# Scalsol/mega.pytorch

Measured on AMD Instinct MI355X. Metric: frames/sec MEGA R-101 inference, 1000x600 VID clip, higher is better.
Workload: dtype bf16

## Files before the change

### include/mega_hip.h

```cpp
#ifndef MEGA_HIP_H
#define MEGA_HIP_H

#include <stddef.h>

#ifdef __cplusplus
extern "C" {
#endif

#define MEGA_F32 0
#define MEGA_BF16 1
#define MEGA_F16 2

#define MEGA_OK 0
#define MEGA_ERR_ARG 1
#define MEGA_ERR_LAUNCH 2
#define MEGA_ERR_WS 3
#define MEGA_ERR_LIMIT 4

int mega_conv2d_nhwc(const void* in, const void* w, const float* scale, const float* bias, const void* residual,
                     void* out, int N, int H, int W, int Cin, int Cout, int R, int S, int stride, int pad, int dil,
                     int relu, int ldo, int ldr, int in_dtype, int out_dtype, void* stream);
int mega_conv2d_nhwc_tile(int M, int Cout, int K);
int mega_conv2d_nhwc_plan(int M, int Cout, int K, int in_dtype);
int mega_conv2d_nhwc_plan_ex(int N, int H, int W, int Cin, int Cout, int R, int S, int stride, int pad, int dil, int ldo,
                             int has_residual, int in_dtype, int out_dtype);

size_t mega_conv2d_nhwc_workspace_bytes(int M, int Cout, int K);
int mega_conv2d_nhwc_ws(const void* in, const void* w, const float* scale, const float* bias, const void* residual,
                        void* out, int N, int H, int W, int Cin, int Cout, int R, int S, int stride, int pad, int dil,
                        int relu, int ldo, int ldr, int in_dtype, int out_dtype, void* ws, size_t ws_bytes, void* stream);

int mega_stem_conv_bn_relu(const float* in, const float* w_tap64, const float* scale, const float* bias, void* out,
                           int N, int H, int W, int out_dtype, void* stream);
int mega_stem_conv_bn_relu_bf16(const float* in, const void* w_n176_bf16, const float* scale, const float* bias,
                                void* out, int N, int H, int W, void* stream);
int mega_stem_conv_bn_relu_bf16_u8(const void* frames_u8, const void* w_n176_bf16, const float* scale, const float* bias,
                                   void* out, int N, int H, int W, float mean0, float mean1, float mean2, int to_bgr,
                                   void* stream);

int mega_stem_pool_dt(const void* in, int u8, const void* w_n176, const float* scale, const float* bias, void* out, int N,
                      int H, int W, float mean0, float mean1, float mean2, int to_bgr, int dtype, void* stream);

int mega_maxpool3x3s2_nhwc(const void* in, void* out, int N, int H, int W, int C, int dtype, void* stream);

int mega_avgpool2x2_ceil_nhwc(const void* in, void* out, int N, int H, int W, int C, int dtype, void* stream);

int mega_roi_align_fwd(const void* feat, const float* rois, void* out, int K, int C, int H, int W,
                       float spatial_scale, int pooled_h, int pooled_w, int sampling_ratio, int in_nhwc,
                       int out_nhwc, int dtype, int out_dtype, void* stream);

size_t mega_nms_full_workspace_bytes(int n);
int mega_nms(const float* dets, const float* scores, int n, float thr, int strict_gt, long long* keep_out,
             int* keep_cnt, void* ws, size_t ws_bytes, void* stream);

size_t mega_nms_workspace_bytes(int P, int nmax);
int mega_nms_sorted(const float* boxes, const int* counts, const unsigned char* valid, const int* order, int P,
                    int nmax, float thr, int strict_gt, int max_keep, int* keep_pos, int* keep_cnt,
                    unsigned char* flags, void* ws, size_t ws_bytes, void* stream);

size_t mega_rpn_select_workspace_bytes(int B, int pre_nms_top_n);
int mega_rpn_select_idx(const float* rpn_out, const float* cell_anchors, int B, int Hf, int Wf, int A, int ldc,
                        int anchor_stride, int pre_nms_top_n, int post_nms_top_n, float nms_thresh, int strict_gt,
                        float min_size, float im_w, float im_h, float* proposals, float* prop_scores, int* prop_cnt,
                        int* prop_index, void* ws, size_t ws_bytes, void* stream);

size_t mega_postprocess_workspace_bytes(int R, int NC);
int mega_postprocess(const float* logits, const float* deltas, const float* props, const int* nprop, int R, int NC,
                     float wx, float wy, float ww, float wh, float im_w, float im_h, float score_thresh,
                     float nms_thresh, int strict_gt, int max_det, float* out_boxes, float* out_scores,
                     long long* out_labels, int* out_cnt, float* probs_out, void* ws, size_t ws_bytes,
                     void* stream);

size_t mega_postprocess_batched_workspace_bytes(int B, int R, int NC);
int mega_postprocess_batched(const float* logits, const float* deltas, const float* props, const int* nprop, int B,
// ... 164 lines not shown
```

### mega/pytorch_amd/_lib.py

```python
import ctypes
import os

HERE = os.path.dirname(os.path.abspath(__file__))
LIB_PATH = os.path.join(HERE, "libmega_hip.so")

c_int, c_float, c_void_p, c_size_t = ctypes.c_int, ctypes.c_float, ctypes.c_void_p, ctypes.c_size_t
c_longlong = ctypes.c_longlong

_ERR = {1: "bad argument", 2: "kernel launch failure", 3: "workspace too small", 4: "kernel loop bound exceeded"}

SIGNATURES = {
    "mega_conv2d_nhwc": (c_int, [c_void_p] * 6 + [c_int] * 15 + [c_void_p]),
    "mega_conv2d_nhwc_ws": (c_int, [c_void_p] * 6 + [c_int] * 15 + [c_void_p, c_size_t, c_void_p]),
    "mega_conv2d_nhwc_workspace_bytes": (c_size_t, [c_int] * 3),
    "mega_stem_conv_bn_relu": (c_int, [c_void_p] * 5 + [c_int] * 4 + [c_void_p]),
    "mega_stem_conv_bn_relu_bf16": (c_int, [c_void_p] * 5 + [c_int] * 3 + [c_void_p]),
    "mega_stem_conv_bn_relu_bf16_u8": (c_int, [c_void_p] * 5 + [c_int] * 3 + [c_float] * 3 + [c_int, c_void_p]),
    "mega_stem_pool_dt": (c_int, [c_void_p, c_int] + [c_void_p] * 4 + [c_int] * 3 + [c_float] * 3 + [c_int, c_int, c_void_p]),
    "mega_maxpool3x3s2_nhwc": (c_int, [c_void_p] * 2 + [c_int] * 5 + [c_void_p]),
    "mega_avgpool2x2_ceil_nhwc": (c_int, [c_void_p] * 2 + [c_int] * 5 + [c_void_p]),
    "mega_roi_align_fwd": (c_int, [c_void_p] * 3 + [c_int] * 4 + [c_float] + [c_int] * 7 + [c_void_p]),
    "mega_nms_full_workspace_bytes": (c_size_t, [c_int]),
    "mega_nms": (c_int, [c_void_p, c_void_p, c_int, c_float, c_int, c_void_p, c_void_p, c_void_p, c_size_t, c_void_p]),
    "mega_nms_workspace_bytes": (c_size_t, [c_int, c_int]),
    "mega_nms_sorted": (c_int, [c_void_p] * 4 + [c_int, c_int, c_float, c_int, c_int] + [c_void_p] * 4 +
                        [c_size_t, c_void_p]),
    "mega_rpn_select_workspace_bytes": (c_size_t, [c_int, c_int]),
    "mega_rpn_select_idx": (c_int, [c_void_p, c_void_p] + [c_int] * 8 + [c_float, c_int, c_float, c_float, c_float] +
                            [c_void_p] * 5 + [c_size_t, c_void_p]),
    "mega_postprocess_workspace_bytes": (c_size_t, [c_int, c_int]),
    "mega_postprocess": (c_int, [c_void_p] * 4 + [c_int, c_int] + [c_float] * 8 + [c_int, c_int] + [c_void_p] * 6 +
                         [c_size_t, c_void_p]),
    "mega_postprocess_batched_workspace_bytes": (c_size_t, [c_int, c_int, c_int]),
    "mega_postprocess_batched": (c_int, [c_void_p] * 4 + [c_int, c_int, c_int] + [c_float] * 8 + [c_int, c_int] +
                                 [c_void_p] * 6 + [c_size_t, c_void_p]),
    "mega_postprocess_candidates_batched": (c_int, [c_void_p] * 4 + [c_int] * 3 + [c_float] * 7 + [c_void_p] * 3),
    "mega_bbox_aug_merge_workspace_bytes": (c_size_t, [c_int] * 4),
    "mega_bbox_aug_merge": (c_int, [c_void_p, c_void_p] + [c_int] * 4 + [c_void_p] * 3 + [c_float, c_float, c_int, c_int] +
                            [c_void_p] * 5 + [c_size_t, c_void_p]),
    "mega_soft_merge_workspace_bytes": (c_size_t, [c_int] * 4),
    "mega_soft_merge": (c_int, [c_void_p, c_void_p] + [c_int] * 4 + [c_void_p] * 3 +
                        [c_float, c_float, c_int, c_int, c_float, c_int, c_float, c_int, c_int] + [c_void_p] * 5 +
                        [c_size_t, c_void_p]),
    "mega_position_logits": (c_int, [c_void_p] * 6 + [c_int] * 4 + [c_void_p]),
    "mega_relation_attention_splits": (c_int, [c_int, c_int, c_int]),
    "mega_relation_attention_workspace_bytes": (c_size_t, [c_int, c_int, c_int]),
    "mega_relation_attention": (c_int, [c_void_p, c_int, c_void_p, c_int, c_void_p, c_int, c_void_p, c_int,
                                        c_void_p, c_int, c_void_p, c_void_p, c_int, c_int, c_int, c_int, c_float,
                                        c_int, c_void_p, c_size_t, c_void_p]),
    "mega_relation_attention_batched": (c_int, [c_void_p, c_int, c_int, c_float, c_int, c_void_p]),
    "mega_position_logits_tiled_dt": (c_int, [c_void_p] * 6 + [c_int] * 3 + [c_void_p]),
# ... 80 lines not shown
```

### mega/pytorch_amd/csrc/spatial.hip

```cpp
#include "common.h"

namespace {

constexpr int ST_T = 16;
constexpr int ST_P = ST_T * 2 + 5;
constexpr int ST_PW = ST_P + 1;

template <typename OT>
__global__ __launch_bounds__(256) void stem_conv_kernel(const float* __restrict__ in, const float* __restrict__ w,
                                                        const float* __restrict__ scale,
                                                        const float* __restrict__ bias, OT* __restrict__ out, int N,
                                                        int H, int W, int Ho, int Wo) {
  __shared__ float patch[3][ST_P][ST_PW];
  const int tid = threadIdx.x;
  const int n = blockIdx.z;
  const int oy0 = blockIdx.y * ST_T, ox0 = blockIdx.x * ST_T;
  const int iy0 = oy0 * 2 - 3, ix0 = ox0 * 2 - 3;
  for (int e = tid; e < 3 * ST_P * ST_P; e += 256) {
    const int c = e / (ST_P * ST_P);
    const int rem = e - c * ST_P * ST_P;
    const int y = rem / ST_P, x = rem - y * ST_P;
    const int iy = iy0 + y, ix = ix0 + x;
    float v = 0.f;
    if ((unsigned)iy < (unsigned)H && (unsigned)ix < (unsigned)W) v = in[((size_t)(n * 3 + c) * H + iy) * W + ix];
// ... 524 lines not shown
    for (int i = 0; i < 2; ++i)
#pragma unroll
      for (int j = 0; j < 2; ++j)
        acc[i][j] = __builtin_amdgcn_mfma_f32_32x32x16_bf16(__builtin_bit_cast(bf16x8_t, a[i]),
                                                            __builtin_bit_cast(bf16x8_t, b[j]), acc[i][j], 0, 0, 0);
  }
  __syncthreads();
#pragma unroll
  for (int j = 0; j < 2; ++j) {
    const int ch = j * 32 + p;
    const float sc = scale[ch], bi = bias[ch];
#pragma unroll
    for (int i = 0; i < 2; ++i) {
#pragma unroll
      for (int r = 0; r < 16; ++r) {
        const int px = (r & 3) + 8 * (r >> 2) + 4 * half;
        *reinterpret_cast<unsigned short*>(smem + ((2 * wave + i) * SM_TX + px) * SM_OUT_PS + ch * 2) =
            (bf16_t)(f32_to_bf16(fmaxf(acc[i][j][r] * sc + bi, 0.f)) & 0x7fffu);
      }
    }
  }
  __syncthreads();
#pragma unroll
  for (int i = 0; i < SM_TY * SM_TX * 8 / 256; ++i) {
    const int v = tid + 256 * i;
    const int pl = v >> 3, cv = v & 7;
    const int oy = oy0 + pl / SM_TX, ox = ox0 + pl % SM_TX;
    if (oy < Ho && ox < Wo)
      *reinterpret_cast<uint4*>(out + (((size_t)n * Ho + oy) * Wo + ox) * 64 + cv * 8) =
          *reinterpret_cast<const uint4*>(smem + pl * SM_OUT_PS + cv * 16);
  }
}

constexpr int SP_PY = 4, SP_PX = 16;
constexpr int SP_TY = 2 * SP_PY + 1, SP_TX = 2 * SP_PX + 1;
constexpr int SP_NPIX = SP_TY * SP_TX;
constexpr int SP_NBLK = (SP_NPIX + 31) / 32;
constexpr int SP_PH = 2 * SP_TY + 5, SP_PW = 2 * SP_TX + 5, SP_PS = 72;
static_assert(SP_PW + 1 <= SP_PS, "the zero-weight 8th tap reads one column past the patch");

__host__ __device__ constexpr int sp_group_off(int g) {
  const int gg = g < 21 ? g : 20;
  return (gg / 7) * (SP_PH * SP_PS) + (gg % 7) * SP_PS;
}

template <bool U8, typename HT = bf16_t>
__global__ __launch_bounds__(256, 3) void stem_pool_kernel(const void* __restrict__ in_, const bf16_t* __restrict__ w,
                                                        const float* __restrict__ scale, const float* __restrict__ bias,
                                                        bf16_t* __restrict__ out, int N, int H, int W, int Ho, int Wo, int Hp,
                                                        int Wp, float m0, float m1, float m2, int to_bgr) {
  const float* __restrict__ in = reinterpret_cast<const float*>(in_);
  const unsigned char* __restrict__ in8 = reinterpret_cast<const unsigned char*>(in_);
  constexpr int PATCH_B = (3 * SP_PH * SP_PS * 2 + 15) / 16 * 16, OUT_PS = 144;
  constexpr int LDS_B = SP_NBLK * 32 * OUT_PS > PATCH_B + 64 * SM_WS * 2 ? SP_NBLK * 32 * OUT_PS : PATCH_B + 64 * SM_WS * 2;
  __shared__ __attribute__((aligned(16))) unsigned char smem[LDS_B];
  unsigned short* patch = reinterpret_cast<unsigned short*>(smem);
  unsigned short* wl = reinterpret_cast<unsigned short*>(smem + PATCH_B);
  const int tid = threadIdx.x, lane = tid & 63, wave = tid >> 6;
  const int n = blockIdx.z;
  const int py0 = blockIdx.y * SP_PY, px0 = blockIdx.x * SP_PX;
  const int oy0 = 2 * py0 - 1, ox0 = 2 * px0 - 1;
  const int iy0 = oy0 * 2 - 3, ix0 = ox0 * 2 - 3;
  constexpr int NPL = (3 * SP_PH * SP_PS + 255) / 256, NWL = (64 * (SM_K / 8) + 255) / 256;
  float pv[NPL];
  u32x4_t wv[NWL];
#pragma unroll
  for (int i = 0; i < NPL; ++i) {
    const int e = tid + 256 * i;
    const int c = e / (SP_PH * SP_PS);
    const int rem = e - c * (SP_PH * SP_PS);
    const int y = rem / SP_PS, x = rem - y * SP_PS;
    const int iy = iy0 + y, ix = ix0 + x;
    pv[i] = 0.f;
    if (e < 3 * SP_PH * SP_PS && x < SP_PW && (unsigned)iy < (unsigned)H && (unsigned)ix < (unsigned)W) {
      if (U8) {
        const float mean = c == 0 ? m0 : (c == 1 ? m1 : m2);
        pv[i] = (float)in8[(((size_t)n * H + iy) * W + ix) * 3 + (to_bgr ? 2 - c : c)] - mean;
      } else {
        pv[i] = in[((size_t)(n * 3 + c) * H + iy) * W + ix];
      }
    }
  }
#pragma unroll
  for (int i = 0; i < NWL; ++i) {
    const int e = tid + 256 * i;
    const int row = e / (SM_K / 8), v = e - row * (SM_K / 8);
    if (e < 64 * (SM_K / 8)) wv[i] = *reinterpret_cast<const u32x4_t*>(w + row * SM_K + v * 8);
  }
#pragma unroll
  for (int i = 0; i < NPL; ++i) {
    const int e = tid + 256 * i;
    if (e < 3 * SP_PH * SP_PS) patch[e] = Half16<HT>::cvt(pv[i]);
  }
#pragma unroll
  for (int i = 0; i < NWL; ++i) {
    const int e = tid + 256 * i;
    const int row = e / (SM_K / 8), v = e - row * (SM_K / 8);
    if (e < 64 * (SM_K / 8)) *reinterpret_cast<u32x4_t*>(&wl[row * SM_WS + v * 8]) = wv[i];
  }
  __syncthreads();

  const int p = lane & 31, half = lane >> 5;
  constexpr int NB = 3;
  f32x16_t acc[NB][2];
  int pbase[NB];
#pragma unroll
  for (int b = 0; b < NB; ++b) {
    const int pix = min(32 * (wave + 4 * b) + p, SP_NPIX - 1);
    const int r = pix / SP_TX, c = pix - r * SP_TX;
    pbase[b] = 2 * r * SP_PS + 2 * c;
#pragma unroll
    for (int j = 0; j < 2; ++j)
#pragma unroll
      for (int q = 0; q < 16; ++q) acc[b][j][q] = 0.f;
  }
#pragma unroll
  for (int ks = 0; ks < SM_K / 16; ++ks) {
    u32x4_t bfr[2];
#pragma unroll
    for (int j = 0; j < 2; ++j) bfr[j] = *reinterpret_cast<const u32x4_t*>(&wl[(j * 32 + p) * SM_WS + ks * 16 + half * 8]);
#pragma unroll
    for (int b = 0; b < NB; ++b) {
      if (wave + 4 * b < SP_NBLK) {
        const unsigned* base = reinterpret_cast<const unsigned*>(patch + pbase[b] + (half ? sp_group_off(2 * ks + 1) : sp_group_off(2 * ks)));
        const u32x4_t a = {base[0], base[1], base[2], base[3]};
#pragma unroll
        for (int j = 0; j < 2; ++j) acc[b][j] = Half16<HT>::mfma32(a, bfr[j], acc[b][j]);
      }
    }
  }
  __syncthreads();
#pragma unroll
  for (int j = 0; j < 2; ++j) {
    const int ch = j * 32 + p;
    const float sc = scale[ch], bi = bias[ch];
#pragma unroll
    for (int b = 0; b < NB; ++b) {
      if (wave + 4 * b < SP_NBLK) {
#pragma unroll
        for (int q = 0; q < 16; ++q) {
          const int pix = 32 * (wave + 4 * b) + (q & 3) + 8 * (q >> 2) + 4 * half;
          const int r = pix / SP_TX, c = pix - r * SP_TX;
          const int oy = oy0 + r, ox = ox0 + c;
          const bool ok = pix < SP_NPIX && (unsigned)oy < (unsigned)Ho && (unsigned)ox < (unsigned)Wo;
          const unsigned short hv = (unsigned short)(Half16<HT>::cvt(fmaxf(acc[b][j][q] * sc + bi, 0.f)) & 0x7fffu);
          *reinterpret_cast<unsigned short*>(smem + pix * OUT_PS + ch * 2) = ok ? hv : (unsigned short)0;
        }
      }
    }
  }
  __syncthreads();
#pragma unroll
  for (int i = 0; i < SP_PY * SP_PX * 8 / 256; ++i) {
    const int v = tid + 256 * i;
    const int pl = v >> 3, cv = v & 7;
    const int ty = pl / SP_PX, tx = pl - ty * SP_PX;
    const int oy = py0 + ty, ox = px0 + tx;
    typedef unsigned short u16x8_t __attribute__((ext_vector_type(8)));
    u16x8_t m = {0, 0, 0, 0, 0, 0, 0, 0};
#pragma unroll
    for (int dy = 0; dy < 3; ++dy)
#pragma unroll
      for (int dx = 0; dx < 3; ++dx) {
        const u16x8_t q = *reinterpret_cast<const u16x8_t*>(smem + ((2 * ty + dy) * SP_TX + 2 * tx + dx) * OUT_PS + cv * 16);
        m = __builtin_elementwise_max(m, q);
      }
    if (oy < Hp && ox < Wp) *reinterpret_cast<u16x8_t*>(out + (((size_t)n * Hp + oy) * Wp + ox) * 64 + cv * 8) = m;
  }
}

}

extern "C" int mega_stem_conv_bn_relu_bf16(const float* in, const void* w_n176_bf16, const float* scale,
                                           const float* bias, void* out, int N, int H, int W, void* stream) {
  mega_clear_error();
  if (!in || !w_n176_bf16 || !scale || !bias || !out || N <= 0 || H <= 0 || W <= 0) return MEGA_ERR_ARG;
  const int Ho = (H + 6 - 7) / 2 + 1, Wo = (W + 6 - 7) / 2 + 1;
  dim3 grid(cdiv(Wo, SM_TX), cdiv(Ho, SM_TY), N);
  hipLaunchKernelGGL(stem_mfma_kernel<false>, grid, dim3(256), 0, (hipStream_t)stream, (const void*)in,
                     (const bf16_t*)w_n176_bf16, scale, bias, (bf16_t*)out, N, H, W, Ho, Wo, 0.f, 0.f, 0.f, 0);
  return mega_check_launch();
}

extern "C" int mega_stem_conv_bn_relu_bf16_u8(const void* frames_u8, const void* w_n176_bf16, const float* scale,
                                              const float* bias, void* out, int N, int H, int W, float mean0, float mean1,
                                              float mean2, int to_bgr, void* stream) {
  mega_clear_error();
  if (!frames_u8 || !w_n176_bf16 || !scale || !bias || !out || N <= 0 || H <= 0 || W <= 0) return MEGA_ERR_ARG;
  const int Ho = (H + 6 - 7) / 2 + 1, Wo = (W + 6 - 7) / 2 + 1;
  dim3 grid(cdiv(Wo, SM_TX), cdiv(Ho, SM_TY), N);
  hipLaunchKernelGGL(stem_mfma_kernel<true>, grid, dim3(256), 0, (hipStream_t)stream, frames_u8, (const bf16_t*)w_n176_bf16,
                     scale, bias, (bf16_t*)out, N, H, W, Ho, Wo, mean0, mean1, mean2, to_bgr);
  return mega_check_launch();
}

extern "C" int mega_stem_conv_bn_relu(const float* in, const float* w_tap64, const float* scale, const float* bias,
                                      void* out, int N, int H, int W, int out_dtype, void* stream) {
  mega_clear_error();
  if (!in || !w_tap64 || !scale || !bias || !out || N <= 0 || H <= 0 || W <= 0) return MEGA_ERR_ARG;
  const int Ho = (H + 6 - 7) / 2 + 1, Wo = (W + 6 - 7) / 2 + 1;
// ... 100 lines not shown
                       (bf16_t*)out, K, C, H, W, spatial_scale, pooled_h, pooled_w, sampling_ratio, in_nhwc, out_nhwc);
  else if (dtype == MEGA_F16 && out_dtype == MEGA_F16)
    hipLaunchKernelGGL((roi_align_kernel<f16_t, f16_t>), grid, dim3(threads), 0, st, (const f16_t*)feat, rois,
                       (f16_t*)out, K, C, H, W, spatial_scale, pooled_h, pooled_w, sampling_ratio, in_nhwc, out_nhwc);
  else if (dtype == MEGA_F32 && out_dtype == MEGA_F32)
    hipLaunchKernelGGL((roi_align_kernel<float, float>), grid, dim3(threads), 0, st, (const float*)feat, rois,
                       (float*)out, K, C, H, W, spatial_scale, pooled_h, pooled_w, sampling_ratio, in_nhwc, out_nhwc);
  else
    return MEGA_ERR_ARG;
  return mega_check_launch();
}

extern "C" int mega_avgpool2x2_ceil_nhwc(const void* in, void* out, int N, int H, int W, int C, int dtype,
                                         void* stream) {
  mega_clear_error();
  if (!in || !out || N <= 0 || H <= 0 || W <= 0 || C <= 0) return MEGA_ERR_ARG;
  const int Ho = (H + 1) / 2, Wo = (W + 1) / 2;
  hipStream_t st = (hipStream_t)stream;
  const int ve = dtype == MEGA_BF16 ? 8 : 4;
  if (C % ve) return MEGA_ERR_ARG;
  const size_t total = (size_t)N * Ho * Wo * (C / ve);
  const int blocks = (int)((total + 255) / 256 > 8192 ? 8192 : (total + 255) / 256);
  if (dtype == MEGA_BF16)
    hipLaunchKernelGGL((avgpool2_kernel<bf16_t>), dim3(blocks), dim3(256), 0, st, (const bf16_t*)in, (bf16_t*)out, N, H,
                       W, C, Ho, Wo);
  else if (dtype == MEGA_F32)
    hipLaunchKernelGGL((avgpool2_kernel<float>), dim3(blocks), dim3(256), 0, st, (const float*)in, (float*)out, N, H, W,
                       C, Ho, Wo);
  else
    return MEGA_ERR_ARG;
  return mega_check_launch();
}

extern "C" int mega_stem_pool_dt(const void* in, int u8, const void* w_n176, const float* scale, const float* bias,
                                 void* out, int N, int H, int W, float mean0, float mean1, float mean2, int to_bgr,
                                 int dtype, void* stream) {
  mega_clear_error();
  if (!in || !w_n176 || !scale || !bias || !out || N <= 0 || H <= 0 || W <= 0) return MEGA_ERR_ARG;
  if (dtype != MEGA_BF16 && dtype != MEGA_F16) return MEGA_ERR_ARG;
  const int Ho = (H + 6 - 7) / 2 + 1, Wo = (W + 6 - 7) / 2 + 1;
  const int Hp = (Ho + 2 - 3) / 2 + 1, Wp = (Wo + 2 - 3) / 2 + 1;
  dim3 grid(cdiv(Wp, SP_PX), cdiv(Hp, SP_PY), N);
  hipStream_t st = (hipStream_t)stream;
  const bf16_t* w = (const bf16_t*)w_n176;
  bf16_t* o = (bf16_t*)out;
  if (!u8) { mean0 = mean1 = mean2 = 0.f; to_bgr = 0; }
  if (dtype == MEGA_F16) {
    if (u8) hipLaunchKernelGGL((stem_pool_kernel<true, f16_t>), grid, dim3(256), 0, st, in, w, scale, bias, o, N, H, W, Ho, Wo, Hp, Wp, mean0, mean1, mean2, to_bgr);
    else hipLaunchKernelGGL((stem_pool_kernel<false, f16_t>), grid, dim3(256), 0, st, in, w, scale, bias, o, N, H, W, Ho, Wo, Hp, Wp, mean0, mean1, mean2, to_bgr);
  } else {
    if (u8) hipLaunchKernelGGL((stem_pool_kernel<true, bf16_t>), grid, dim3(256), 0, st, in, w, scale, bias, o, N, H, W, Ho, Wo, Hp, Wp, mean0, mean1, mean2, to_bgr);
    else hipLaunchKernelGGL((stem_pool_kernel<false, bf16_t>), grid, dim3(256), 0, st, in, w, scale, bias, o, N, H, W, Ho, Wo, Hp, Wp, mean0, mean1, mean2, to_bgr);
  }
  return mega_check_launch();
}

extern "C" int mega_roi_align_fwd_planes_dt(const float* feat, const float* rois, void* out, int K, int C, int H, int W,
                                            float spatial_scale, int pooled_h, int pooled_w, int sampling_ratio, int dtype,
                                            void* stream) {
  mega_clear_error();
  if (K == 0) return MEGA_OK;
  if (dtype != MEGA_BF16 && dtype != MEGA_F16) return MEGA_ERR_ARG;
  if (!feat || !rois || !out || K < 0 || C <= 0 || C % 4 || H <= 0 || W <= 0 || pooled_h <= 0 || pooled_w <= 0) return MEGA_ERR_ARG;
  const int CV = C / 4;
  const long long total = (long long)K * pooled_h * pooled_w * CV;
  const bool sliced = CV % 8 == 0 && CV / 8 >= 16 && total / 8 >= 256 * 64;
  long long nb = ((sliced ? total / 8 : total) + 255) / 256;
  if (nb > 131072) nb = 131072;
  dim3 vgrid((unsigned)(sliced ? nb * 8 : nb));
  hipStream_t st = (hipStream_t)stream;
  const bool separable = sliced && sampling_ratio <= 0 && pooled_w <= RS_MAXPW && pooled_h <= RS_MAXPW;
  if (separable) {
    if (dtype == MEGA_F16)
      hipLaunchKernelGGL((roi_align_nhwc_sep_kernel<float, 8, true, f16_t>), dim3((unsigned)(K * 8)), dim3(256), 0, st, feat, rois,
                         (float*)out, K, C, H, W, spatial_scale, pooled_h, pooled_w);
    else
      hipLaunchKernelGGL((roi_align_nhwc_sep_kernel<float, 8, true, bf16_t>), dim3((unsigned)(K * 8)), dim3(256), 0, st, feat, rois,
                         (float*)out, K, C, H, W, spatial_scale, pooled_h, pooled_w);
    return mega_check_launch();
  }
  if (dtype == MEGA_F16) {
    if (sliced)
      hipLaunchKernelGGL((roi_align_nhwc_vec_kernel<float, true, true, f16_t>), vgrid, dim3(256), 0, st, feat, rois, (float*)out, K, C,
                         H, W, spatial_scale, pooled_h, pooled_w, sampling_ratio);
    else
      hipLaunchKernelGGL((roi_align_nhwc_vec_kernel<float, false, true, f16_t>), vgrid, dim3(256), 0, st, feat, rois, (float*)out, K,
                         C, H, W, spatial_scale, pooled_h, pooled_w, sampling_ratio);
// ... 10 lines not shown
```

### mega/pytorch_amd/ops.py

```python
import contextlib
import ctypes
import threading
import math

import torch

from . import _lib

F32, BF16, F16 = 0, 1, 2
_DT = {torch.float32: F32, torch.bfloat16: BF16, torch.float16: F16}
_HALF = (torch.bfloat16, torch.float16)


def _dt(t):
    try:
        return _DT[t.dtype]
    except KeyError:
        raise TypeError("unsupported dtype %s (float32 / bfloat16 / float16 only)" % t.dtype)


_LAUNCH = threading.local()


def _stream():
# ... 289 lines not shown
    assert C == 3 and x_nchw.dtype == torch.float32 and x_nchw.is_contiguous()
    Ho, Wo = (H - 1) // 2 + 1, (W - 1) // 2 + 1
    out = torch.empty((N, Ho, Wo, 64), dtype=out_dtype, device=x_nchw.device)
    _tok = _pb("stem", 2.0 * N * Ho * Wo * 64 * 147, x_nchw.numel() * 4 + out.numel() * out.element_size())
    if out_dtype == torch.bfloat16 and w_n160 is not None:
        _gpu(w_n160)
        assert w_n160.dtype == torch.bfloat16 and tuple(w_n160.shape) == (64, 176) and w_n160.is_contiguous()
        rc = lib.mega_stem_conv_bn_relu_bf16(_ptr(x_nchw), _ptr(w_n160), _ptr(scale), _ptr(bias), _ptr(out), N, H, W,
                                             _stream())
    else:
        rc = lib.mega_stem_conv_bn_relu(_ptr(x_nchw), _ptr(w_tap64), _ptr(scale), _ptr(bias), _ptr(out), N, H, W,
                                        _DT[out_dtype], _stream())
    _pe(_tok)
    _lib.check(rc, "mega_stem_conv_bn_relu")
    return out


def stem_u8(frames_u8, w_n160, scale, bias, mean, to_bgr=True):
    _gpu(frames_u8, w_n160, scale, bias)
    lib = _lib.load()
    N, H, W, C = frames_u8.shape
    assert C == 3 and frames_u8.dtype == torch.uint8 and frames_u8.is_contiguous()
    assert w_n160.dtype == torch.bfloat16 and tuple(w_n160.shape) == (64, 176) and w_n160.is_contiguous()
    Ho, Wo = (H - 1) // 2 + 1, (W - 1) // 2 + 1
    out = torch.empty((N, Ho, Wo, 64), dtype=torch.bfloat16, device=frames_u8.device)
    _tok = _pb("stem", 2.0 * N * Ho * Wo * 64 * 147, frames_u8.numel() + out.numel() * 2)
    rc = lib.mega_stem_conv_bn_relu_bf16_u8(_ptr(frames_u8), _ptr(w_n160), _ptr(scale), _ptr(bias), _ptr(out), N, H, W,
                                            float(mean[0]), float(mean[1]), float(mean[2]), int(to_bgr), _stream())
    _pe(_tok)
    _lib.check(rc, "mega_stem_conv_bn_relu_bf16_u8")
    return out


def stem_pool(x, w_n160, scale, bias, mean=None, to_bgr=True):
    _gpu(x, w_n160, scale, bias)
    lib = _lib.load()
    u8 = x.dtype == torch.uint8
    if u8:
        N, H, W, C = x.shape
        assert mean is not None
    else:
        N, C, H, W = x.shape
        assert x.dtype == torch.float32
        mean = (0.0, 0.0, 0.0)
    assert C == 3 and x.is_contiguous()
    assert w_n160.dtype in _HALF and tuple(w_n160.shape) == (64, 176) and w_n160.is_contiguous()
    Ho, Wo = (H - 1) // 2 + 1, (W - 1) // 2 + 1
    Hp, Wp = (Ho - 1) // 2 + 1, (Wo - 1) // 2 + 1
    out = torch.empty((N, Hp, Wp, 64), dtype=w_n160.dtype, device=x.device)
    _tok = _pb("stem", 2.0 * N * Ho * Wo * 64 * 147, x.numel() * x.element_size() + out.numel() * 2)
    rc = lib.mega_stem_pool_dt(_ptr(x), int(u8), _ptr(w_n160), _ptr(scale), _ptr(bias), _ptr(out), N, H, W,
                               float(mean[0]), float(mean[1]), float(mean[2]), int(to_bgr), _dt(w_n160), _stream())
    _pe(_tok)
    _lib.check(rc, "mega_stem_pool_dt")
    return out


def pack_stem_weight_bf16(w_oihw, dtype=torch.bfloat16):
    w = torch.zeros((64, 22, 8), dtype=torch.float32, device=w_oihw.device)
    w[:, :21, :7] = w_oihw.detach().float().reshape(64, 21, 7)
    w = w.reshape(64, 176)
    return w.to(dtype).contiguous()


def maxpool3x3s2(x):
    _gpu(x)
    lib = _lib.load()
    N, H, W, C = x.shape
    assert x.is_contiguous()
    Ho, Wo = (H - 1) // 2 + 1, (W - 1) // 2 + 1
    out = torch.empty((N, Ho, Wo, C), dtype=x.dtype, device=x.device)
    _tok = _pb("maxpool", 0.0, (x.numel() + out.numel()) * x.element_size())
    rc = lib.mega_maxpool3x3s2_nhwc(_ptr(x), _ptr(out), N, H, W, C, _dt(x), _stream())
    _pe(_tok)
    _lib.check(rc, "mega_maxpool3x3s2_nhwc")
    return out


def roi_align(feat, rois, spatial_scale, pooled, sampling_ratio, in_nhwc=True, out_nhwc=True):
    _gpu(feat, rois)
    lib = _lib.load()
    if in_nhwc:
        B, H, W, C = feat.shape
    else:
        B, C, H, W = feat.shape
    ph, pw = pooled
    K = rois.shape[0]
# ... 995 lines not shown
```

Before: 903.0.

## Make fused stem conv+maxpool persistent with double-buffered patch prefetch

Turns the fused stem conv/BN/ReLU/maxpool kernel into a persistent grid sized to twice the CU count. Each block loops over tiles and prefetches the next tile's input patch into a second LDS buffer while running MFMA on the current one. It also reshapes tiles to 7x8 pooled outputs, uses 16-byte vector loads with byte alignment for uint8 frames, keeps scale and bias in LDS, and reserves separate LDS regions for the patch and output staging. The cost is more dynamic LDS per block, which caps occupancy at two blocks per CU, plus more complex boundary handling. The stem is only a small part of the R-101 MEGA pipeline, so its effect on the end-to-end rate is limited.

```diff
diff --git a/include/mega_hip.h b/include/mega_hip.h
--- a/include/mega_hip.h
+++ b/include/mega_hip.h
@@ -40,6 +40,9 @@
 
 int mega_stem_pool_dt(const void* in, int u8, const void* w_n176, const float* scale, const float* bias, void* out, int N,
                       int H, int W, float mean0, float mean1, float mean2, int to_bgr, int dtype, void* stream);
+int mega_stem_pool_dt_grid(const void* in, int u8, const void* w_n176, const float* scale, const float* bias, void* out, int N,
+                           int H, int W, float mean0, float mean1, float mean2, int to_bgr, int dtype, int max_blocks,
+                           void* stream);
 
 int mega_maxpool3x3s2_nhwc(const void* in, void* out, int N, int H, int W, int C, int dtype, void* stream);
 
diff --git a/mega/pytorch_amd/_lib.py b/mega/pytorch_amd/_lib.py
--- a/mega/pytorch_amd/_lib.py
+++ b/mega/pytorch_amd/_lib.py
@@ -17,6 +17,7 @@
     "mega_stem_conv_bn_relu_bf16": (c_int, [c_void_p] * 5 + [c_int] * 3 + [c_void_p]),
     "mega_stem_conv_bn_relu_bf16_u8": (c_int, [c_void_p] * 5 + [c_int] * 3 + [c_float] * 3 + [c_int, c_void_p]),
     "mega_stem_pool_dt": (c_int, [c_void_p, c_int] + [c_void_p] * 4 + [c_int] * 3 + [c_float] * 3 + [c_int, c_int, c_void_p]),
+    "mega_stem_pool_dt_grid": (c_int, [c_void_p, c_int] + [c_void_p] * 4 + [c_int] * 3 + [c_float] * 3 + [c_int, c_int, c_int, c_void_p]),
     "mega_maxpool3x3s2_nhwc": (c_int, [c_void_p] * 2 + [c_int] * 5 + [c_void_p]),
     "mega_avgpool2x2_ceil_nhwc": (c_int, [c_void_p] * 2 + [c_int] * 5 + [c_void_p]),
     "mega_roi_align_fwd": (c_int, [c_void_p] * 3 + [c_int] * 4 + [c_float] + [c_int] * 7 + [c_void_p]),
diff --git a/mega/pytorch_amd/csrc/spatial.hip b/mega/pytorch_amd/csrc/spatial.hip
--- a/mega/pytorch_amd/csrc/spatial.hip
+++ b/mega/pytorch_amd/csrc/spatial.hip
@@ -580,140 +580,250 @@
   }
 }
 
-constexpr int SP_PY = 4, SP_PX = 16;
+constexpr int SP_PY = 7, SP_PX = 8;
 constexpr int SP_TY = 2 * SP_PY + 1, SP_TX = 2 * SP_PX + 1;
 constexpr int SP_NPIX = SP_TY * SP_TX;
 constexpr int SP_NBLK = (SP_NPIX + 31) / 32;
-constexpr int SP_PH = 2 * SP_TY + 5, SP_PW = 2 * SP_TX + 5, SP_PS = 72;
+constexpr int SP_NB = SP_NBLK / 4;
+static_assert(SP_NBLK % 4 == 0, "the MFMA blocks divide evenly over the four waves");
+constexpr int SP_PH = 2 * SP_TY + 5, SP_PW = 2 * SP_TX + 5, SP_PS = 40;
 static_assert(SP_PW + 1 <= SP_PS, "the zero-weight 8th tap reads one column past the patch");
+static_assert(SP_PS % 4 == 0, "a patch row is whole 4-pixel groups");
+constexpr int SP_GR = SP_PS / 4, SP_NIT = SP_PH * SP_GR;
+constexpr int SP_NEL = 3 * SP_PH * SP_PS;
+constexpr int SP_PATCH_B = SP_NEL * 2, SP_OUT_PS = 144;
+static_assert(SP_PATCH_B % 16 == 0, "patch buffers stay 16-byte aligned");
+constexpr int SP_OFF_SC = 64 * SM_WS * 2, SP_OFF_BI = SP_OFF_SC + 256, SP_OFF_P = SP_OFF_BI + 256;
+constexpr int SP_OFF_ST = SP_OFF_P + 2 * SP_PATCH_B, SP_LDS = SP_OFF_ST + SP_NBLK * 32 * SP_OUT_PS;
+static_assert(SP_OFF_P % 16 == 0 && SP_OFF_ST % 16 == 0, "16-byte LDS vectors");
+constexpr int SP_BLOCKS_PER_CU = 2;
+static_assert(SP_BLOCKS_PER_CU * SP_LDS <= 160 * 1024, "two blocks per CU");
 
 __host__ __device__ constexpr int sp_group_off(int g) {
   const int gg = g < 21 ? g : 20;
   return (gg / 7) * (SP_PH * SP_PS) + (gg % 7) * SP_PS;
 }
 
+typedef unsigned int u32x2_t __attribute__((ext_vector_type(2)));
+
 template <bool U8, typename HT = bf16_t>
-__global__ __launch_bounds__(256, 3) void stem_pool_kernel(const void* __restrict__ in_, const bf16_t* __restrict__ w,
-                                                        const float* __restrict__ scale, const float* __restrict__ bias,
-                                                        bf16_t* __restrict__ out, int N, int H, int W, int Ho, int Wo, int Hp,
-                                                        int Wp, float m0, float m1, float m2, int to_bgr) {
+__global__ __launch_bounds__(256, SP_BLOCKS_PER_CU) void stem_pool_kernel(
+    const void* __restrict__ in_, long long in_bytes, const bf16_t* __restrict__ w, const float* __restrict__ scale,
+    const float* __restrict__ bias, bf16_t* __restrict__ out, int N, int H, int W, int Ho, int Wo, int Hp, int Wp, float m0,
+    float m1, float m2, int to_bgr, int tiles_y, int tiles_x, int tiles) {
   const float* __restrict__ in = reinterpret_cast<const float*>(in_);
   const unsigned char* __restrict__ in8 = reinterpret_cast<const unsigned char*>(in_);
-  constexpr int PATCH_B = (3 * SP_PH * SP_PS * 2 + 15) / 16 * 16, OUT_PS = 144;
-  constexpr int LDS_B = SP_NBLK * 32 * OUT_PS > PATCH_B + 64 * SM_WS * 2 ? SP_NBLK * 32 * OUT_PS : PATCH_B + 64 * SM_WS * 2;
-  __shared__ __attribute__((aligned(16))) unsigned char smem[LDS_B];
-  unsigned short* patch = reinterpret_cast<unsigned short*>(smem);
-  unsigned short* wl = reinterpret_cast<unsigned short*>(smem + PATCH_B);
+  extern __shared__ __attribute__((aligned(16))) unsigned char sp_smem[];
+  unsigned short* wl = reinterpret_cast<unsigned short*>(sp_smem);
+  const float* lsc = reinterpret_cast<const float*>(sp_smem + SP_OFF_SC);
+  const float* lbi = reinterpret_cast<const float*>(sp_smem + SP_OFF_BI);
+  unsigned char* stage = sp_smem + SP_OFF_ST;
   const int tid = threadIdx.x, lane = tid & 63, wave = tid >> 6;
-  const int n = blockIdx.z;
-  const int py0 = blockIdx.y * SP_PY, px0 = blockIdx.x * SP_PX;
-  const int oy0 = 2 * py0 - 1, ox0 = 2 * px0 - 1;
-  const int iy0 = oy0 * 2 - 3, ix0 = ox0 * 2 - 3;
-  constexpr int NPL = (3 * SP_PH * SP_PS + 255) / 256, NWL = (64 * (SM_K / 8) + 255) / 256;
-  float pv[NPL];
-  u32x4_t wv[NWL];
-#pragma unroll
-  for (int i = 0; i < NPL; ++i) {
-    const int e = tid + 256 * i;
-    const int c = e / (SP_PH * SP_PS);
-    const int rem = e - c * (SP_PH * SP_PS);
-    const int y = rem / SP_PS, x = rem - y * SP_PS;
-    const int iy = iy0 + y, ix = ix0 + x;
-    pv[i] = 0.f;
-    if (e < 3 * SP_PH * SP_PS && x < SP_PW && (unsigned)iy < (unsigned)H && (unsigned)ix < (unsigned)W) {
-      if (U8) {
-        const float mean = c == 0 ? m0 : (c == 1 ? m1 : m2);
-        pv[i] = (float)in8[(((size_t)n * H + iy) * W + ix) * 3 + (to_bgr ? 2 - c : c)] - mean;
-      } else {
-        pv[i] = in[((size_t)(n * 3 + c) * H + iy) * W + ix];
-      }
-    }
-  }
-#pragma unroll
-  for (int i = 0; i < NWL; ++i) {
+  const int p = lane & 31, half = lane >> 5;
+  const int mis = (int)(reinterpret_cast<uintptr_t>(in_) & 3);
+
+  auto origin = [&](int t, int& n, int& py0, int& px0) {
+    n = t / (tiles_y * tiles_x);
+    const int r = t - n * (tiles_y * tiles_x);
+    const int ty = r / tiles_x;
+    py0 = ty * SP_PY;
+    px0 = (r - ty * tiles_x) * SP_PX;
+  };
+  auto ld_bytes = [&](long long o) -> unsigned {
+    unsigned v = 0;
+#pragma unroll
+    for (int b = 0; b < 4; ++b)
+      if (o + b >= 0 && o + b < in_bytes) v |= (unsigned)in8[o + b] << (8 * b);
+    return v;
+  };
+
+  constexpr int NRAW = U8 ? 8 : (SP_NEL + 255) / 256;
+  constexpr int NRAWV = (NRAW + 3) / 4;
+  auto load_raw = [&](int t, u32x4_t (&raw)[NRAWV]) {
+    int n, py0, px0;
+    origin(t, n, py0, px0);
+    const int iy0 = 4 * py0 - 5, ix0 = 4 * px0 - 5;
+    if constexpr (U8) {
+      long long a0s[2];
+      bool slow[2];
+#pragma unroll
+      for (int i = 0; i < 2; ++i) {
+        const int id = tid + 256 * i;
+        const int y = id / SP_GR, g = id - y * SP_GR;
+        const int iy = iy0 + y, x0 = ix0 + 4 * g;
+        const bool need = id < SP_NIT && (unsigned)iy < (unsigned)H && x0 + 4 > 0 && x0 < W;
+        const long long a = (((long long)n * H + iy) * W + x0) * 3 + mis;
+        const long long a0 = a - (a & 3) - mis;
+        const bool whole = need && a0 >= 0 && a0 + 16 <= in_bytes;
+        a0s[i] = a0;
+        slow[i] = need && !whole;
+        raw[i] = u32x4_t{0u, 0u, 0u, 0u};
+        if (whole) {
+          const unsigned* q = reinterpret_cast<const unsigned*>(in8 + a0);
+          raw[i] = u32x4_t{q[0], q[1], q[2], q[3]};
+        }
+      }
+      if (slow[0] || slow[1]) {
+#pragma unroll
+        for (int i = 0; i < 2; ++i)
+          if (slow[i]) raw[i] = u32x4_t{ld_bytes(a0s[i]), ld_bytes(a0s[i] + 4), ld_bytes(a0s[i] + 8), ld_bytes(a0s[i] + 12)};
+      }
+    } else {
+#pragma unroll
+      for (int i = 0; i < NRAW; ++i) {
+        const int e = tid + 256 * i;
+        const int c = e / (SP_PH * SP_PS);
+        const int rem = e - c * (SP_PH * SP_PS);
+        const int y = rem / SP_PS, x = rem - y * SP_PS;
+        const int iy = iy0 + y, ix = ix0 + x;
+        raw[(i) >> 2][(i) & 3] = 0u;
+        if (e < SP_NEL && x < SP_PW && (unsigned)iy < (unsigned)H && (unsigned)ix < (unsigned)W)
+          raw[(i) >> 2][(i) & 3] = __float_as_uint(in[((size_t)(n * 3 + c) * H + iy) * W + ix]);
+      }
+    }
+  };
+  auto store_patch = [&](int t, const u32x4_t (&raw)[NRAWV], unsigned short* patch) {
+    if constexpr (U8) {
+      int n, py0, px0;
+      origin(t, n, py0, px0);
+      const int iy0 = 4 * py0 - 5, ix0 = 4 * px0 - 5;
+#pragma unroll
+      for (int i = 0; i < 2; ++i) {
+        const int id = tid + 256 * i;
+        const int y = id / SP_GR, g = id - y * SP_GR;
+        const int iy = iy0 + y, x0 = ix0 + 4 * g;
+        const bool rowok = (unsigned)iy < (unsigned)H;
+        const unsigned sh = (((unsigned)(n * H + iy) * (unsigned)W + (unsigned)x0) * 3u + (unsigned)mis) & 3u;
+        unsigned by[3];
+#pragma unroll
+        for (int k = 0; k < 3; ++k) by[k] = __builtin_amdgcn_alignbyte(raw[i][k + 1], raw[i][k], sh);
+        if (id < SP_NIT) {
+#pragma unroll
+          for (int bc = 0; bc < 3; ++bc) {
+            const int c = to_bgr ? 2 - bc : bc;
+            const float mean = to_bgr ? (bc == 0 ? m2 : (bc == 1 ? m1 : m0)) : (bc == 0 ? m0 : (bc == 1 ? m1 : m2));
+            float v[4];
+#pragma unroll
+            for (int q = 0; q < 4; ++q) {
+              const int b = 3 * q + bc;
+              const float src = (float)((by[b >> 2] >> (8 * (b & 3))) & 0xffu);
+              const bool ok = rowok && (unsigned)(x0 + q) < (unsigned)W;
+              v[q] = ok ? src - mean : 0.f;
+            }
+            const u32x2_t pk = {(unsigned)Half16<HT>::cvt(v[0]) | ((unsigned)Half16<HT>::cvt(v[1]) << 16),
+                                (unsigned)Half16<HT>::cvt(v[2]) | ((unsigned)Half16<HT>::cvt(v[3]) << 16)};
+            *reinterpret_cast<u32x2_t*>(patch + (c * SP_PH + y) * SP_PS + 4 * g) = pk;
+          }
+        }
+      }
+    } else {
+#pragma unroll
+      for (int i = 0; i < NRAW; ++i) {
+        const int e = tid + 256 * i;
+        if (e < SP_NEL) patch[e] = Half16<HT>::cvt(__uint_as_float(raw[(i) >> 2][(i) & 3]));
+      }
+    }
+  };
+
+#pragma unroll
+  for (int i = 0; i < (64 * (SM_K / 8) + 255) / 256; ++i) {
     const int e = tid + 256 * i;
     const int row = e / (SM_K / 8), v = e - row * (SM_K / 8);
-    if (e < 64 * (SM_K / 8)) wv[i] = *reinterpret_cast<const u32x4_t*>(w + row * SM_K + v * 8);
-  }
-#pragma unroll
-  for (int i = 0; i < NPL; ++i) {
-    const int e = tid + 256 * i;
-    if (e < 3 * SP_PH * SP_PS) patch[e] = Half16<HT>::cvt(pv[i]);
-  }
-#pragma unroll
-  for (int i = 0; i < NWL; ++i) {
-    const int e = tid + 256 * i;
-    const int row = e / (SM_K / 8), v = e - row * (SM_K / 8);
-    if (e < 64 * (SM_K / 8)) *reinterpret_cast<u32x4_t*>(&wl[row * SM_WS + v * 8]) = wv[i];
-  }
-  __syncthreads();
-
-  const int p = lane & 31, half = lane >> 5;
-  constexpr int NB = 3;
-  f32x16_t acc[NB][2];
-  int pbase[NB];
-#pragma unroll
-  for (int b = 0; b < NB; ++b) {
-    const int pix = min(32 * (wave + 4 * b) + p, SP_NPIX - 1);
-    const int r = pix / SP_TX, c = pix - r * SP_TX;
+    if (e < 64 * (SM_K / 8))
+      *reinterpret_cast<u32x4_t*>(&wl[row * SM_WS + v * 8]) = *reinterpret_cast<const u32x4_t*>(w + row * SM_K + v * 8);
+  }
+  if (tid < 64) *reinterpret_cast<float*>(sp_smem + SP_OFF_SC + tid * 4) = scale[tid];
+  else if (tid < 128) *reinterpret_cast<float*>(sp_smem + SP_OFF_BI + (tid - 64) * 4) = bias[tid - 64];
+
+  int pbase[SP_NB], prow[SP_NB], pcol[SP_NB];
+#pragma unroll
+  for (int b = 0; b < SP_NB; ++b) {
+    const int pix = 32 * (wave + 4 * b) + p;
+    const int pc = min(pix, SP_NPIX - 1);
+    const int r = pc / SP_TX, c = pc - r * SP_TX;
     pbase[b] = 2 * r * SP_PS + 2 * c;
-#pragma unroll
-    for (int j = 0; j < 2; ++j)
-#pragma unroll
-      for (int q = 0; q < 16; ++q) acc[b][j][q] = 0.f;
-  }
-#pragma unroll
-  for (int ks = 0; ks < SM_K / 16; ++ks) {
-    u32x4_t bfr[2];
-#pragma unroll
-    for (int j = 0; j < 2; ++j) bfr[j] = *reinterpret_cast<const u32x4_t*>(&wl[(j * 32 + p) * SM_WS + ks * 16 + half * 8]);
-#pragma unroll
-    for (int b = 0; b < NB; ++b) {
-      if (wave + 4 * b < SP_NBLK) {
-        const unsigned* base = reinterpret_cast<const unsigned*>(patch + pbase[b] + (half ? sp_group_off(2 * ks + 1) : sp_group_off(2 * ks)));
-        const u32x4_t a = {base[0], base[1], base[2], base[3]};
-#pragma unroll
-        for (int j = 0; j < 2; ++j) acc[b][j] = Half16<HT>::mfma32(a, bfr[j], acc[b][j]);
-      }
-    }
-  }
-  __syncthreads();
-#pragma unroll
-  for (int j = 0; j < 2; ++j) {
-    const int ch = j * 32 + p;
-    const float sc = scale[ch], bi = bias[ch];
-#pragma unroll
-    for (int b = 0; b < NB; ++b) {
-      if (wave + 4 * b < SP_NBLK) {
-#pragma unroll
-        for (int q = 0; q < 16; ++q) {
-          const int pix = 32 * (wave + 4 * b) + (q & 3) + 8 * (q >> 2) + 4 * half;
-          const int r = pix / SP_TX, c = pix - r * SP_TX;
-          const int oy = oy0 + r, ox = ox0 + c;
-          const bool ok = pix < SP_NPIX && (unsigned)oy < (unsigned)Ho && (unsigned)ox < (unsigned)Wo;
-          const unsigned short hv = (unsigned short)(Half16<HT>::cvt(fmaxf(acc[b][j][q] * sc + bi, 0.f)) & 0x7fffu);
-          *reinterpret_cast<unsigned short*>(smem + pix * OUT_PS + ch * 2) = ok ? hv : (unsigned short)0;
+    prow[b] = pix < SP_NPIX ? r : -0x40000000;
+    pcol[b] = c;
+  }
+
+  u32x4_t raw[NRAWV];
+  int cur = 1;
+  for (int t = (int)blockIdx.x - (int)gridDim.x; t < tiles; t += gridDim.x) {
+    const int tn = t + gridDim.x;
+    const unsigned short* patch = reinterpret_cast<const unsigned short*>(sp_smem + SP_OFF_P + cur * SP_PATCH_B);
+    unsigned short* patch_next = reinterpret_cast<unsigned short*>(sp_smem + SP_OFF_P + (cur ^ 1) * SP_PATCH_B);
+    int n, py0, px0;
+    origin(t, n, py0, px0);
+    const int oy0 = 2 * py0 - 1, ox0 = 2 * px0 - 1;
+    const int tl = min(tn, tiles - 1);
+    load_raw(tl, raw);
+    if (t >= 0) {
+      f32x16_t acc[SP_NB][2];
+#pragma unroll
+      for (int b = 0; b < SP_NB; ++b)
+#pragma unroll
+        for (int j = 0; j < 2; ++j)
+#pragma unroll
+          for (int q = 0; q < 16; ++q) acc[b][j][q] = 0.f;
+#pragma unroll
+      for (int ks = 0; ks < SM_K / 16; ++ks) {
+        u32x4_t wf[2];
+#pragma unroll
+        for (int j = 0; j < 2; ++j) wf[j] = *reinterpret_cast<const u32x4_t*>(&wl[(j * 32 + p) * SM_WS + ks * 16 + half * 8]);
+#pragma unroll
+        for (int b = 0; b < SP_NB; ++b) {
+          const unsigned* base = reinterpret_cast<const unsigned*>(patch + pbase[b] + (half ? sp_group_off(2 * ks + 1) : sp_group_off(2 * ks)));
+          const u32x4_t a = {base[0], base[1], base[2], base[3]};
+#pragma unroll
+          for (int j = 0; j < 2; ++j) acc[b][j] = Half16<HT>::mfma32(wf[j], a, acc[b][j]);
         }
       }
-    }
-  }
-  __syncthreads();
-#pragma unroll
-  for (int i = 0; i < SP_PY * SP_PX * 8 / 256; ++i) {
-    const int v = tid + 256 * i;
-    const int pl = v >> 3, cv = v & 7;
-    const int ty = pl / SP_PX, tx = pl - ty * SP_PX;
-    const int oy = py0 + ty, ox = px0 + tx;
-    typedef unsigned short u16x8_t __attribute__((ext_vector_type(8)));
-    u16x8_t m = {0, 0, 0, 0, 0, 0, 0, 0};
-#pragma unroll
-    for (int dy = 0; dy < 3; ++dy)
-#pragma unroll
-      for (int dx = 0; dx < 3; ++dx) {
-        const u16x8_t q = *reinterpret_cast<const u16x8_t*>(smem + ((2 * ty + dy) * SP_TX + 2 * tx + dx) * OUT_PS + cv * 16);
-        m = __builtin_elementwise_max(m, q);
-      }
-    if (oy < Hp && ox < Wp) *reinterpret_cast<u16x8_t*>(out + (((size_t)n * Hp + oy) * Wp + ox) * 64 + cv * 8) = m;
+      unsigned keep[SP_NB];
+#pragma unroll
+      for (int b = 0; b < SP_NB; ++b)
+        keep[b] = (unsigned)(oy0 + prow[b]) < (unsigned)Ho && (unsigned)(ox0 + pcol[b]) < (unsigned)Wo ? 0x7fff7fffu : 0u;
+#pragma unroll
+      for (int j = 0; j < 2; ++j)
+#pragma unroll
+        for (int g = 0; g < 4; ++g) {
+          const int ch = j * 32 + 8 * g + 4 * half;
+          const f32x4_t sc = *reinterpret_cast<const f32x4_t*>(lsc + ch), bi = *reinterpret_cast<const f32x4_t*>(lbi + ch);
+#pragma unroll
+          for (int b = 0; b < SP_NB; ++b) {
+            float r[4];
+#pragma unroll
+            for (int e = 0; e < 4; ++e)
+              r[e] = fmaxf(fmaf(acc[b][j][4 * g + e], sc[e], bi[e]), 0.f);
+            const u32x2_t v = {Half16<HT>::pack2(r[0], r[1]) & keep[b], Half16<HT>::pack2(r[2], r[3]) & keep[b]};
+            *reinterpret_cast<u32x2_t*>(stage + (32 * (wave + 4 * b) + p) * SP_OUT_PS + ch * 2) = v;
+          }
+        }
+    }
+    store_patch(tl, raw, patch_next);
+    __syncthreads();
+#pragma unroll
+    for (int i = 0; i < (SP_PY * SP_PX * 8 + 255) / 256; ++i) {
+      const int v = tid + 256 * i;
+      const int pl = v >> 3, cv = v & 7;
+      const int ty = pl / SP_PX, tx = pl - ty * SP_PX;
+      const int oy = py0 + ty, ox = px0 + tx;
+      if (t >= 0 && v < SP_PY * SP_PX * 8 && oy < Hp && ox < Wp) {
+        typedef unsigned short u16x8_t __attribute__((ext_vector_type(8)));
+        u16x8_t q[9];
+#pragma unroll
+        for (int dy = 0; dy < 3; ++dy)
+#pragma unroll
+          for (int dx = 0; dx < 3; ++dx)
+            q[3 * dy + dx] = *reinterpret_cast<const u16x8_t*>(stage + ((2 * ty + dy) * SP_TX + 2 * tx + dx) * SP_OUT_PS + cv * 16);
+        asm volatile("" ::: "memory");
+        u16x8_t m = q[0];
+#pragma unroll
+        for (int k = 1; k < 9; ++k) m = __builtin_elementwise_max(m, q[k]);
+        *reinterpret_cast<u16x8_t*>(out + (((size_t)n * Hp + oy) * Wp + ox) * 64 + cv * 8) = m;
+      }
+    }
+    __syncthreads();
+    cur ^= 1;
   }
 }
 
@@ -880,27 +990,58 @@
   return mega_check_launch();
 }
 
-extern "C" int mega_stem_pool_dt(const void* in, int u8, const void* w_n176, const float* scale, const float* bias,
-                                 void* out, int N, int H, int W, float mean0, float mean1, float mean2, int to_bgr,
-                                 int dtype, void* stream) {
+extern "C" int mega_stem_pool_dt_grid(const void* in, int u8, const void* w_n176, const float* scale, const float* bias,
+                                      void* out, int N, int H, int W, float mean0, float mean1, float mean2, int to_bgr,
+                                      int dtype, int max_blocks, void* stream) {
   mega_clear_error();
-  if (!in || !w_n176 || !scale || !bias || !out || N <= 0 || H <= 0 || W <= 0) return MEGA_ERR_ARG;
+  if (!in || !w_n176 || !scale || !bias || !out || N <= 0 || H <= 0 || W <= 0 || max_blocks < 0) return MEGA_ERR_ARG;
   if (dtype != MEGA_BF16 && dtype != MEGA_F16) return MEGA_ERR_ARG;
   const int Ho = (H + 6 - 7) / 2 + 1, Wo = (W + 6 - 7) / 2 + 1;
   const int Hp = (Ho + 2 - 3) / 2 + 1, Wp = (Wo + 2 - 3) / 2 + 1;
-  dim3 grid(cdiv(Wp, SP_PX), cdiv(Hp, SP_PY), N);
+  const int ty = cdiv(Hp, SP_PY), tx = cdiv(Wp, SP_PX);
+  const long long tiles = (long long)N * ty * tx;
+  if (tiles > 0x7FFFFFFF - 65536 || (long long)N * 3 > 0x7FFFFFFF) return MEGA_ERR_ARG;
+  int cus = 256;
+  {
+    static int cached[64] = {0};
+    int dev = 0, n = 0;
+    if (hipGetDevice(&dev) != hipSuccess || dev < 0 || dev >= 64) dev = 0;
+    if (!cached[dev]) {
+      if (hipDeviceGetAttribute(&n, hipDeviceAttributeMultiprocessorCount, dev) == hipSuccess && n > 0) cached[dev] = n;
+      else cached[dev] = 256;
+    }
+    cus = cached[dev];
+  }
+  long long grid = (long long)SP_BLOCKS_PER_CU * cus;
+  if (grid > 65536) grid = 65536;
+  if (tiles < grid) grid = tiles;
+  if (max_blocks > 0 && max_blocks < grid) grid = max_blocks;
   hipStream_t st = (hipStream_t)stream;
   const bf16_t* w = (const bf16_t*)w_n176;
   bf16_t* o = (bf16_t*)out;
   if (!u8) { mean0 = mean1 = mean2 = 0.f; to_bgr = 0; }
+  const long long in_bytes = (long long)N * H * W * 3 * (u8 ? 1 : 4);
+#define MEGA_SP_LAUNCH(U8_, HT_)                                                                                             \
+  do {                                                                                                                       \
+    (void)hipFuncSetAttribute((const void*)stem_pool_kernel<U8_, HT_>, hipFuncAttributeMaxDynamicSharedMemorySize, SP_LDS);  \
+    hipLaunchKernelGGL((stem_pool_kernel<U8_, HT_>), dim3((unsigned)grid), dim3(256), SP_LDS, st, in, in_bytes, w, scale,    \
+                       bias, o, N, H, W, Ho, Wo, Hp, Wp, mean0, mean1, mean2, to_bgr, ty, tx, (int)tiles);                   \
+  } while (0)
   if (dtype == MEGA_F16) {
-    if (u8) hipLaunchKernelGGL((stem_pool_kernel<true, f16_t>), grid, dim3(256), 0, st, in, w, scale, bias, o, N, H, W, Ho, Wo, Hp, Wp, mean0, mean1, mean2, to_bgr);
-    else hipLaunchKernelGGL((stem_pool_kernel<false, f16_t>), grid, dim3(256), 0, st, in, w, scale, bias, o, N, H, W, Ho, Wo, Hp, Wp, mean0, mean1, mean2, to_bgr);
+    if (u8) MEGA_SP_LAUNCH(true, f16_t);
+    else MEGA_SP_LAUNCH(false, f16_t);
   } else {
-    if (u8) hipLaunchKernelGGL((stem_pool_kernel<true, bf16_t>), grid, dim3(256), 0, st, in, w, scale, bias, o, N, H, W, Ho, Wo, Hp, Wp, mean0, mean1, mean2, to_bgr);
-    else hipLaunchKernelGGL((stem_pool_kernel<false, bf16_t>), grid, dim3(256), 0, st, in, w, scale, bias, o, N, H, W, Ho, Wo, Hp, Wp, mean0, mean1, mean2, to_bgr);
-  }
+    if (u8) MEGA_SP_LAUNCH(true, bf16_t);
+    else MEGA_SP_LAUNCH(false, bf16_t);
+  }
+#undef MEGA_SP_LAUNCH
   return mega_check_launch();
+}
+
+extern "C" int mega_stem_pool_dt(const void* in, int u8, const void* w_n176, const float* scale, const float* bias,
+                                 void* out, int N, int H, int W, float mean0, float mean1, float mean2, int to_bgr,
+                                 int dtype, void* stream) {
+  return mega_stem_pool_dt_grid(in, u8, w_n176, scale, bias, out, N, H, W, mean0, mean1, mean2, to_bgr, dtype, 0, stream);
 }
 
 extern "C" int mega_roi_align_fwd_planes_dt(const float* feat, const float* rois, void* out, int K, int C, int H, int W,
diff --git a/mega/pytorch_amd/ops.py b/mega/pytorch_amd/ops.py
--- a/mega/pytorch_amd/ops.py
+++ b/mega/pytorch_amd/ops.py
@@ -345,7 +345,7 @@
     return out
 
 
-def stem_pool(x, w_n160, scale, bias, mean=None, to_bgr=True):
+def stem_pool(x, w_n160, scale, bias, mean=None, to_bgr=True, max_blocks=0):
     _gpu(x, w_n160, scale, bias)
     lib = _lib.load()
     u8 = x.dtype == torch.uint8
@@ -362,10 +362,11 @@
     Hp, Wp = (Ho - 1) // 2 + 1, (Wo - 1) // 2 + 1
     out = torch.empty((N, Hp, Wp, 64), dtype=w_n160.dtype, device=x.device)
     _tok = _pb("stem", 2.0 * N * Ho * Wo * 64 * 147, x.numel() * x.element_size() + out.numel() * 2)
-    rc = lib.mega_stem_pool_dt(_ptr(x), int(u8), _ptr(w_n160), _ptr(scale), _ptr(bias), _ptr(out), N, H, W,
-                               float(mean[0]), float(mean[1]), float(mean[2]), int(to_bgr), _dt(w_n160), _stream())
-    _pe(_tok)
-    _lib.check(rc, "mega_stem_pool_dt")
+    rc = lib.mega_stem_pool_dt_grid(_ptr(x), int(u8), _ptr(w_n160), _ptr(scale), _ptr(bias), _ptr(out), N, H, W,
+                                    float(mean[0]), float(mean[1]), float(mean[2]), int(to_bgr), _dt(w_n160),
+                                    int(max_blocks), _stream())
+    _pe(_tok)
+    _lib.check(rc, "mega_stem_pool_dt_grid")
     return out
 
 
```

New measurement: 908.9 (median of 6 runs). No clear change (+0.7%).
